# mbed92/soft-grip

Hardware: AMD Instinct MI355X
Metric: env steps/sec (whole node) at batch=4096 (higher is better)
Workload: dtype f64; 1 GPU; configs[2]: 4096 envs/GPU, softbox scene (nv=118), stiffness ~ U(300,1400), reference 200-step squeeze schedule from reset, 7 substeps per env step; 327 equality rows (composite neighbour equalities on: DESIGN.md 2, U2); volume tendon damper integrated explicitly; envs_per_gpu=4096, envs_flagged_bad=0

## Files before the change

soft-grip_amd/csrc/sg_phase.hip:

```cpp
#include "sg_work.h"

struct GenLds {
  StageRec2* stage;
  double* gas;
  double* gg;
  double* tmp;
  const double (*boxp)[3];
  const double (*boxm)[9];
  const ChainKin* K;
  const ChainLds2* cs;
  const double *qe, *ve, *asme, *we;
};

__device__ __forceinline__ void sg_gen_capsule(const SgPhaseArgs& a, const GenLds& L, int e, double* cp, double* cax) {
  const int N = a.nelem;
  auto EL = [&](int f, int k) { return a.elem[(size_t)f * N + k]; };
  const double dq = L.qe[e] - EL(SGE_QPOS0, e);
  cp[0] = EL(SGE_GX, e) + EL(SGE_AX, e) * dq; cp[1] = EL(SGE_GY, e) + EL(SGE_AY, e) * dq; cp[2] = EL(SGE_GZ, e) + EL(SGE_AZ, e) * dq;
  cax[0] = EL(SGE_CX, e); cax[1] = EL(SGE_CY, e); cax[2] = EL(SGE_CZ, e);
}

__device__ __noinline__ int sg_gen_phase(const SgPhaseArgs& a, const SgPlanHeader& H, const int env, const GenLds L, int* flags, int* touch) {
  const int lane = threadIdx.x, N = a.nelem;
  auto EL = [&](int f, int k) { return a.elem[(size_t)f * N + k]; };
// ... 621 lines not shown
              double fld[SG_RK];
#pragma unroll
              for (int q = 0; q < SG_RK; q++) fld[q] = 0.0;
              if (r < 3) {
#pragma unroll
                for (int d = 0; d < SG_CD; d++) fld[d] = c.Jf[r][d];
                fld[4] = c.Js[r]; fld[5] = c.b[r]; fld[6] = c.f[r];
                fld[7] = Afull[r][0] * c.f[0] + Afull[r][1] * c.f[1] + Afull[r][2] * c.f[2];
                fld[8] = Afull[r][0]; fld[9] = Afull[r][1]; fld[10] = Afull[r][2];
                fld[11] = c.invm * c.Js[r];
                fld[15] = c.R;
              } else {
                fld[0] = P11; fld[1] = P12; fld[2] = P22; fld[4] = __hiloint2double(0, sl);
                fld[8] = ee1; fld[9] = ee2; fld[10] = ecs; fld[11] = esn;
              }
              fld[12] = Wm[0][r]; fld[13] = Wm[1][r]; fld[14] = Wm[2][r];
#pragma unroll
              for (int pr = 0; pr < SG_RK / 2; pr++) fp[r][pr] = make_double2(fld[2 * pr], fld[2 * pr + 1]);
            }
          }
          if (!a.rowlayout) {
          double* ro = W.crec + SG_REC_INDEX(i, env / SG_EPW, 0, 2 * (env % SG_EPW) + half, nwb);
#pragma unroll
          for (int r = 0; r < 3; r++)
#pragma unroll
            for (int d = 0; d < SG_CD; d++) ro[(4 * r + d) * SG_SPW] = c.Jf[r][d];
#pragma unroll
          for (int r = 0; r < 3; r++) ro[(12 + r) * SG_SPW] = c.Js[r];
#pragma unroll
          for (int q = 0; q < 6; q++) ro[(15 + q) * SG_SPW] = c.A[q];
#pragma unroll
          for (int r = 0; r < 3; r++) ro[(21 + r) * SG_SPW] = c.b[r];
          ro[24 * SG_SPW] = c.R;
          ro[25 * SG_SPW] = c.invm;
#pragma unroll
          for (int r = 0; r < 3; r++) ro[(26 + r) * SG_SPW] = c.f[r];
          ((int*)(ro + 29 * SG_SPW))[0] = sl;
          }
        }
        const int nk = (ns0 > ns1 ? ns0 : ns1) - 32 * k;
        if (a.rowlayout && nk > 0) {
          const int nwb8 = (a.nenv + 7) / 8;
          const int li = lane & 31;
          auto X = [&](int sl_, int L) -> double2* {
            return (double2*)&Sm.stage[sl_ >> 4][32 * k] + ((sl_ & 15) * 8 + L);
          };
          __syncthreads();
          double2* const e0 = (double2*)&Sm.stage[li >> 4][32 * k] + ((li & 15) * 8 + 4 * half);
#pragma unroll
          for (int pr = 0; pr < SG_RK / 2; pr++) {
            e0[0] = fp[0][pr]; e0[1] = fp[1][pr]; e0[2] = fp[2][pr]; e0[3] = fp[3][pr];
            __syncthreads();
#pragma unroll
            for (int j = 0; j < 4; j++) {
              if (8 * j >= nk) break;
              const int e = j * 64 + lane, s_ = e >> 3, L = e & 7;
              if (s_ < nk) *(double2*)(W.crow + SG_ROW_INDEX(32 * k + s_, env >> 3, 2 * pr, 8 * (env & 7) + L, nwb8)) = *X(s_, L);
            }
            __syncthreads();
          }
        }
      }
      SG_T(5);
      double eqR[R], eqb[R], eqf[R];
      double tbp = 0, tjp = 0, tAp = 0;
#pragma unroll
      for (int r = 0; r < R; r++) {
        int e = r * 64 + lane;
        eqR[r] = 1; eqb[r] = 0; eqf[r] = 0;
        if (e < N) {
          double pos = qe[r] - EL(SGE_QPOS0, e), imp = impedance(H.eqj_solimp, pos, 0);
          eqR[r] = fmax(SG_MINVAL, (1 - imp) / imp * EL(SGE_INVW, e));
          double aref = -H.eqj_B * ve[r] - H.eqj_K * imp * pos;
          eqb[r] = asme[r] - aref;
          eqf[r] = -(we[r] - aref) / eqR[r];
          tbp += coef[r] * asme[r]; tjp += coef[r] * we[r]; tAp += coef[r] * coef[r] * invm[r];
        }
      }
      const int nnb = NB ? H.nnb : 0;
      constexpr int ND = NB ? 3 : 0;
      int nbe2[R][3], nbid[R][3];
      double nbc0[R][3];
      [[maybe_unused]] double nbff[R][3];
      [[maybe_unused]] double* const gnbf = W.nbf + (size_t)env * 3 * N;
#pragma unroll
      for (int r = 0; r < R; r++)
#pragma unroll
        for (int d = 0; d < 3; d++) { nbe2[r][d] = -1; nbid[r][d] = -1; nbc0[r][d] = 0; nbff[r][d] = 0; }
      if constexpr (NB) {
        const double im0 = 1.0 / (EL(SGE_MASS, 0) + EL(SGE_ARMATURE, 0));
        const SG_CONSTAS int* const cposc = (const SG_CONSTAS int*)a.cpos;
        const bool wantc = a.rowlayout && a.cst_rounds;
#pragma unroll
        for (int r = 0; r < R; r++) {
          const int e = r * 64 + lane;
          if (e < N) {
            double c4[4] = {0.0, 0.0, 0.0, 0.0};
            if (wantc) c4[0] = sg_div(im0, im0 + eqR[r]);
#pragma unroll
            for (int d = 0; d < 3; d++) {
              const int e2 = nbtabc[d * N + e];
              if (e2 >= 0) {
                const int id = nbtabc[(3 + d) * N + e];
                const double pos = (qe[r] - EL(SGE_QPOS0, e)) - (Sm.as[e2] - EL(SGE_QPOS0, e2)), imp = impedance(H.eqj_solimp, pos, 0);
                const double Rr = fmax(SG_MINVAL, (1 - imp) / imp * (EL(SGE_INVW, e) + EL(SGE_INVW, e2)));
                const double aref = -H.eqj_B * (ve[r] - Sm.ve[e2]) - H.eqj_K * imp * pos;
                const double bb = (asme[r] - Sm.asme[e2]) - aref, ff = -((we[r] - Sm.we[e2]) - aref) / Rr;
                nbe2[r][d] = e2; nbid[r][d] = id; nbc0[r][d] = ff * (0.5 * Rr * ff + bb);
                nbff[r][d] = ff; gnbf[id] = ff;
                W.nbb[(size_t)env * 3 * N + id] = bb; W.nbR[(size_t)env * 3 * N + id] = Rr;
                if (wantc) c4[1 + d] = sg_div(im0, 2.0 * im0 + Rr);
              }
            }
            if (wantc) {
              double* const dst = W.cst + SG_CST_INDEX(env >> 2, 0, 16 * (env & 3), a.cst_rounds) + cposc[e];
              *(double2*)dst = make_double2(c4[0], c4[1]);
              *(double2*)(dst + 2) = make_double2(c4[2], c4[3]);
            }
          }
        }
      }
      const double tpos = L0 - H.t0_L0, timp = impedance(H.eqt_solimp, tpos, 0), tR = fmax(SG_MINVAL, (1 - timp) / timp * H.eqt_invw);
      const double taref = -H.eqt_B * Ld - H.eqt_K * timp * tpos;
      const double tb = wave_sum2(tbp) - taref, tjar = wave_sum2(tjp) - taref, tA = wave_sum2(tAp) + tR;
      double tf = -tjar / tR;
      const int nmaxs = ns0 > ns1 ? ns0 : ns1;

      double aF[SG_CD];
      auto recompute_a = [&]() {
        __syncthreads();
#pragma unroll
        for (int r = 0; r < R; r++) {
          int e = r * 64 + lane;
          if (e < N) {
            double fe = eqf[r] + coef[r] * tf;
            if constexpr (NB) {
#pragma unroll
              for (int d = 0; d < 3; d++) if (nbid[r][d] >= 0) fe += nbff[r][d];
              double fin[3];
#pragma unroll
              for (int d = 0; d < 3; d++) { const int ii = nbtabc[(6 + d) * N + e]; fin[d] = ii >= 0 ? gnbf[ii] : 0.0; }
#pragma unroll
              for (int d = 0; d < 3; d++) fe -= fin[d];
            }
            double as_ = invm[r] * fe;
#pragma unroll
            for (int cb = 0; cb < SG_MAXCH * SG_CG; cb++) {
              const int u = Sm.eslot[e][cb], i0 = u & 0x3F, nst = u >> 6;
              if (nst >= 1) as_ += cval_at(cb / SG_CG, i0);
              if (nst >= 2) as_ += cval_at(cb / SG_CG, i0 + 1);
            }
            if constexpr (GEN)
              if (ngen) as_ += GL.gas[e];
            Sm.as[e] = as_;
          }
        }
        __syncthreads();
        double g[SG_CD] = {0, 0, 0, 0};
#pragma unroll
        for (int k = 0; k < CPL; k++)
#pragma unroll
          for (int d = 0; d < SG_CD; d++) g[d] += cg[k][d];
        if (is_chain_lane) {
          const int la = CS.lim_active;
#pragma unroll
          for (int k = 0; k < SG_MAXLIM; k++)
            if (la >> k & 1) g[k / 2] += CS.lim_sign[k] * CS.lim_f[k];
          if constexpr (GEN)
            if (ngen) {
#pragma unroll
              for (int d = 0; d < SG_CD; d++) g[d] += GL.gg[half * SG_CD + d];
            }
        }
#pragma unroll
        for (int d = 0; d < SG_CD; d++) {
          double x = g[d];
#pragma unroll
          for (int o = 16; o > 0; o >>= 1) x += __shfl_xor(x, o);
          g[d] = x;
        }
#pragma unroll
        for (int a2 = 0; a2 < SG_CD; a2++) {
          double s2 = 0;
#pragma unroll
          for (int b2 = 0; b2 < SG_CD; b2++) s2 += CS.Minv[4 * a2 + b2] * g[b2];
          aF[a2] = s2;
        }
        __syncthreads();
      };
      recompute_a();
      SG_T(6);
      {
        double cp = 0, tJap = 0;
#pragma unroll
        for (int r = 0; r < R; r++) {
          int e = r * 64 + lane;
          if (e < N) {
            double ae = Sm.as[e]; cp += eqf[r] * (0.5 * (ae + eqR[r] * eqf[r]) + eqb[r]); tJap += coef[r] * ae;
#pragma unroll
            for (int d = 0; d < ND; d++)
              if (nbid[r][d] >= 0) cp += 0.5 * nbff[r][d] * (ae - Sm.as[nbe2[r][d]]) + nbc0[r][d];
          }
        }
        double tJa = wave_sum2(tJap);
        if (lane == 0) cp += tf * (0.5 * (tJa + tR * tf) + tb);
        if (is_chain_lane) {
          const int la = CS.lim_active;
#pragma unroll
          for (int k = 0; k < SG_MAXLIM; k++)
            if (la >> k & 1) cp += CS.lim_f[k] * (0.5 * (CS.lim_sign[k] * aF[k / 2] + CS.lim_R[k] * CS.lim_f[k]) + CS.lim_b[k]);
        }
#pragma unroll
        for (int k = 0; k < CPL; k++)
          if ((lane & 31) + 32 * k < myn) {
            double as_ = csl_[k] >= 0 ? Sm.as[csl_[k]] : 0.0, ga = 0;
#pragma unroll
            for (int d = 0; d < SG_CD; d++) ga += cg[k][d] * aF[d];
            cp += 0.5 * (ga + cjsf[k] * as_) + ccost0[k];
          }
        [[maybe_unused]] double aF2[SG_MAXCH][SG_CD];
        if constexpr (GEN)
          if (ngen) {
#pragma unroll
            for (int d = 0; d < SG_CD; d++) {
              const double other = __shfl_xor(aF[d], 32);
              aF2[0][d] = high ? other : aF[d]; aF2[1][d] = high ? aF[d] : other;
            }
            cp += sg_gen_cost(a, env, ngen, aF2, Sm.as, 0);
          }
        double cost = wave_sum2(cp);
        if (cost > 0) {
          if constexpr (GEN)
            if (ngen) {
              sg_gen_cost(a, env, ngen, aF2, Sm.as, 1);
              for (int e = lane; e < N; e += 64) GL.gas[e] = 0.0;
              if (lane < SG_MAXCH * SG_CD) GL.gg[lane] = 0.0;
            }
#pragma unroll
          for (int r = 0; r < R; r++) {
            eqf[r] = 0;
#pragma unroll
            for (int d = 0; d < ND; d++) if (nbid[r][d] >= 0) { nbff[r][d] = 0.0; gnbf[nbid[r][d]] = 0.0; }
          }
          tf = 0;
          if (is_chain_lane) {
#pragma unroll
            for (int k = 0; k < SG_MAXLIM; k++) CS.lim_f[k] = 0;
          }
#pragma unroll
          for (int k = 0; k < CPL; k++) {
            int i = (lane & 31) + 32 * k;
            cjsf[k] = 0;
#pragma unroll
            for (int d = 0; d < SG_CD; d++) cg[k][d] = 0;
            if (i < myn) {
              cval_at(half, i) = 0.0;
              if (!a.rowlayout) {
              double* ro = W.crec + SG_REC_INDEX(i, env / SG_EPW, 0, 2 * (env % SG_EPW) + half, nwb);
#pragma unroll
              for (int r = 0; r < 3; r++) ro[(26 + r) * SG_SPW] = 0.0;
              }
              if (a.rowlayout) {
#pragma unroll
                for (int r = 0; r < 3; r++)
                  *(double2*)(W.crow + SG_ROW_INDEX(i, env >> 3, 6, 8 * (env & 7) + 4 * half + r, (a.nenv + 7) / 8)) = make_double2(0.0, 0.0);
              }
            }
          }
          __syncthreads();
          recompute_a();
        }
      }
      SG_T(7);
#pragma unroll
      for (int r = 0; r < R; r++) {
        int e = r * 64 + lane;
        if (e < N) {
          size_t o = (size_t)env * N + e;
          W.as[o] = Sm.as[e]; W.eqf[o] = eqf[r]; W.eqb[o] = eqb[r]; W.eqR[o] = eqR[r];
        }
      }
      if (is_chain_lane) {
        W.ns[st] = myn < SG_CAP ? myn : SG_CAP;
        W.lim_active[st] = CS.lim_active;
      }
      if (half < nchain) {
        static_assert(4 * SG_MAXLIM == 32, "one limit value per lane of a half");
        const int i = lane & 31;
        W.lim[(size_t)i * S + st] = (&CS.lim_sign[0])[i];
        if (i < SG_CD) W.saF[(size_t)i * S + st] = i == 0 ? aF[0] : (i == 1 ? aF[1] : (i == 2 ? aF[2] : aF[3]));
      }
      if (lane == 0) {
        W.envh[(size_t)0 * a.nenv + env] = tb; W.envh[(size_t)1 * a.nenv + env] = tR;
        W.envh[(size_t)2 * a.nenv + env] = tA; W.envh[(size_t)3 * a.nenv + env] = tf;
        W.shared[env] = shared_slider;
        W.pending[env] = 1;
        W.ncon[env] = ns0 + ns1 + ngen;
        W.gen[env] = ngen;
        W.nefc[env] = N + nnb + 1 + 3 * (ns0 + ns1 + ngen) + __popc(Sm.cs[0].lim_active) + (nchain > 1 ? __popc(Sm.cs[1].lim_active) : 0);
        W.touch[env] = touch;
      }
    }
  }

  SG_T(8);
  __syncthreads();
#pragma unroll
  for (int r = 0; r < R; r++) {
    int e = r * 64 + lane;
    if (e < N) { gq[e0 + e] = qe[r]; gv[e0 + e] = ve[r]; gw[e0 + e] = we[r]; }
  }
  if (lane == 0) {
    if (status | flags) atomicOr(&W.status[env], status | flags);
  }
  SG_T(9);
  SG_TEND();
}

#ifndef SG_X_PHASE_OCC
#define SG_X_PHASE_OCC 2
#endif
#ifndef SG_X_CPL
#define SG_X_CPL 2
#endif
template <int R, int CPL, bool NB, bool GEN = false>
__global__ __launch_bounds__(64, SG_X_PHASE_OCC) void sg_phase_kernel(SgPhaseArgs a) {
  if constexpr (GEN) {
    const int cnt = a.w.gen_count[0];
    a.do_finish = 0; a.do_reset = 0; a.sens = nullptr;
    for (int i = blockIdx.x; i < cnt && i < a.nenv; i += gridDim.x) {
      sg_phase_env<R, CPL, NB, true>(a, a.w.gen_list[i]);
      __syncthreads();
    }
  } else {
    sg_phase_env<R, CPL, NB, false>(a, blockIdx.x);
  }
}

__global__ __launch_bounds__(64) void sg_chain_kernel(SgPhaseArgs a) {
  const int lane = threadIdx.x, c = blockIdx.x & 1, env = (int)(blockIdx.x >> 1) * 64 + lane;
  if (blockIdx.x == 0 && lane == 0) a.w.gen_count[0] = 0;
  SG_T0();
  const SG_CONSTAS SgPlanHeader& H = *(const SG_CONSTAS SgPlanHeader*)a.H;
  const int nv = a.nv, nu = a.nu;
  const size_t S = 2 * (size_t)a.nenv;
  if (env >= a.nenv) return;
  const size_t st = 2 * (size_t)env + c;
  if (a.mask && !a.mask[env]) return;
  SgWork& W = a.w;
  if (a.first && c == 0) { W.status[env] = 0; if (!a.do_finish) W.pending[env] = 0; }
  if (c >= a.nchain) return;
  const int status = a.first ? 0 : W.status[env];
  const int pend = a.do_finish ? W.pending[env] : 0;
  const SgChain& C = H.chain[c];
  const double h = a.timestep;
  double* gq = a.qpos + (size_t)env * nv;
  double* gv = a.qvel + (size_t)env * nv;
  double* gw = a.warm + (size_t)env * nv;
  const double kenv = a.kenv[env];
  double q[SG_CD], v[SG_CD], w[SG_CD], kk[SG_CD], act = 0, ctrl = 0;
#pragma unroll
  for (int d = 0; d < SG_CD; d++) {
// ... 180 lines not shown
```

soft-grip_amd/csrc/sg_rows.hip:

```cpp
#include "sg_work.h"

template <int CTRL>
__device__ __forceinline__ double sg_dpp(double x) {
  int lo = __double2loint(x), hi = __double2hiint(x);
  lo = __builtin_amdgcn_update_dpp(0, lo, CTRL, 0xF, 0xF, true);
  hi = __builtin_amdgcn_update_dpp(0, hi, CTRL, 0xF, 0xF, true);
  return __hiloint2double(hi, lo);
}
template <int R_>
__device__ __forceinline__ double sg_qb(double x) { return sg_dpp<R_ * 0x55>(x); }
__device__ __forceinline__ double sg_qsum(double x) {
  x += sg_dpp<0xB1>(x);
  x += sg_dpp<0x4E>(x);
  return x;
}

__device__ __forceinline__ double sg_gsum8(double x) {
  x = sg_qsum(x);
  x += sg_dpp<0x141>(x);
  return x;
}

__device__ __forceinline__ double sg_gsum16(double x) {
  x = sg_gsum8(x);
  x += sg_dpp<0x140>(x);
  return x;
}

template <int NSL, int NB, int EPW>
__global__ __launch_bounds__(64) void sg_pgs_rows_kernel(SgPgsArgs a) {
  extern __shared__ double lds[];
  static_assert(!NB || EPW == 4, "neighbour-row models: four envs of 16 lanes per wavefront");
  constexpr bool CST = NB == 2;
  constexpr int LSH = NB ? 4 : 3, LPE = 1 << LSH;
  const int lane = threadIdx.x, le = lane >> LSH, g = lane & (LPE - 1), c = g >> 2, r = g & 3;
  const bool in_wave = le < EPW;
  const int lec = in_wave ? le : 0;
  const int env = blockIdx.x * EPW + le;
  const SG_CONSTAS SgPlanHeader& H = *(const SG_CONSTAS SgPlanHeader*)a.H;
  const int N = H.nelem;
  const size_t S = 2 * (size_t)a.nenv;
  const int nwb = (a.nenv + 7) / 8;
  const SgWork& W = a.w;
  const double mu0 = H.con_mu[0], mu1 = H.con_mu[1], pgs_scale = H.pgs_scale, tolerance = H.tolerance;
  const double mur = r == 1 ? mu0 : mu1;
  const double rsel0 = r == 0 ? 1.0 : 0.0, rsel1 = r == 1 ? 1.0 : 0.0, rsel2 = r == 2 ? 1.0 : 0.0;
  const int max_iter = H.iterations;
  unsigned pendmask = 0;
#pragma unroll
  for (int e2 = 0; e2 < EPW; e2++) {
    const int env2 = blockIdx.x * EPW + e2;
    pendmask |= (env2 < a.nenv && W.pending[env2 < a.nenv ? env2 : 0] != 0) ? 1u << e2 : 0u;
  }
  const bool valid = in_wave && ((pendmask >> lec) & 1u) != 0;
  if (pendmask == 0) return;
  constexpr int NR = 8 * NSL;
  constexpr int NA = NR + 8;
  const int NAr = SG_ROWS_NA_NB(N);
  const int GW = (CST ? 4 : 8) * (N + 1);
  double2* const AF = (double2*)lds + (size_t)lec * NR;
  double2* const BR = (double2*)lds + (size_t)EPW * NR + (size_t)lec * NR;
  double* const RI = lds + (size_t)4 * EPW * NR + (size_t)lec * NR;
  double2* const IC = (double2*)(lds + (size_t)5 * EPW * NR);
  double* const Ae = lds + (size_t)lec * NAr;
  double* const GS = lds + (size_t)EPW * NAr + (size_t)lec * GW;
  unsigned* const TAB = (unsigned*)(lds + (size_t)EPW * NAr + (size_t)EPW * GW);
  constexpr int TABW = CST ? 1 : 2;
  double* const Lnb = lds + (size_t)EPW * NAr + (size_t)EPW * GW + (size_t)8 * TABW * (H.eq_rounds + 8);
  double* Lzero = NB ? Lnb : lds + (size_t)(5 * EPW + 2) * NR;
  double* const Lenv = Lnb + 72;
  double* const ASb = NB ? Ae : (double*)AF;
  constexpr int ASS = NB ? 1 : 2;
  if (lane == 0) Lzero[0] = 0.0;
  if constexpr (!NB)
  for (int j = lane; j < NR; j += 64)
    IC[j] = j < N ? make_double2(1.0 / (a.elem[(size_t)SGE_MASS * N + j] + a.elem[(size_t)SGE_ARMATURE * N + j]), a.elem[(size_t)SGE_COEF * N + j]) : make_double2(0.0, 0.0);
#pragma unroll
  for (int e2 = 0; e2 < EPW; e2++) {
    const int env2 = blockIdx.x * EPW + e2;
    const bool v2 = ((pendmask >> e2) & 1u) != 0;
    if constexpr (!NB) {
      double2* const AF2 = (double2*)lds + (size_t)e2 * NR;
      double2* const BR2 = (double2*)lds + (size_t)EPW * NR + (size_t)e2 * NR;
      double* const RI2 = lds + (size_t)4 * EPW * NR + (size_t)e2 * NR;
#pragma unroll
      for (int j0 = 0; j0 < NR; j0 += 64) {
        const int j = j0 + lane;
        double2 af = make_double2(0.0, 0.0), br = make_double2(0.0, 1.0);
        double ri = 0.0;
        if (v2 && j < N) {
          const size_t o = (size_t)env2 * N + j;
          const double Rr = W.eqR[o], im = 1.0 / (a.elem[(size_t)SGE_MASS * N + j] + a.elem[(size_t)SGE_ARMATURE * N + j]);
          af = make_double2(W.as[o], W.eqf[o]); br = make_double2(W.eqb[o], Rr);
          ri = sg_div(1.0, im + Rr);
        }
        if (j < NR) { AF2[j] = af; BR2[j] = br; RI2[j] = ri; }
      }
    } else {
      double* const A2 = lds + (size_t)e2 * NAr;
      double ssum = 0.0;
#pragma unroll
      for (int j0 = 0; j0 < NA; j0 += 64) {
        const int j = j0 + lane;
        const double av = (v2 && j < N) ? W.as[(size_t)env2 * N + j] : 0.0;
        if (j < NAr) A2[j] = av;
        ssum += av;
      }
      ssum = wave_sum2(ssum);
      if (lane == 0) { Lenv[e2] = ssum; Lenv[EPW + e2] = 0.0; }
    }
  }
  if constexpr (NB) {
    [[maybe_unused]] const double im0s = 1.0 / (a.elem[(size_t)SGE_MASS * N] + a.elem[(size_t)SGE_ARMATURE * N]);
    constexpr int REC_TRIPS = (4 * (NR + 1) + 63) / 64;
#pragma unroll 4
    for (int t = 0; t < REC_TRIPS; t++) {
      const int u = lane + 64 * t;
      if (u >= 4 * (N + 1)) continue;
      const int e = u >> 2, d = u & 3, ec = e < N ? e : 0;
      const bool fix = d == 0;
      const int tabw = a.nbtab[(fix ? 0 : d - 1) * N + ec];
      const bool have = e < N && (fix || tabw >= 0);
      double bb[EPW], Rr[EPW], ff[EPW];
#pragma unroll
      for (int e2 = 0; e2 < EPW; e2++) {
        const int env2 = blockIdx.x * EPW + e2, envc = env2 < a.nenv ? env2 : 0;
        const size_t o = fix ? (size_t)envc * N + ec : (size_t)envc * 3 * N + (size_t)(d - 1) * N + ec;
        bb[e2] = (fix ? W.eqb : W.nbb)[o]; Rr[e2] = (fix ? W.eqR : W.nbR)[o]; ff[e2] = (fix ? W.eqf : W.nbf)[o];
      }
#pragma unroll
      for (int e2 = 0; e2 < EPW; e2++) {
        const int env2 = blockIdx.x * EPW + e2;
        const bool v2 = ((pendmask >> e2) & 1u) != 0;
        double* const GS2 = lds + (size_t)EPW * NAr + (size_t)e2 * GW;
        const double gg = (v2 && have) ? bb[e2] + Rr[e2] * ff[e2] : 0.0;
        if constexpr (CST) GS2[u] = gg;
        else ((double2*)GS2)[u] = make_double2(gg, (v2 && have) ? sg_div(im0s, (fix ? im0s : 2.0 * im0s) + Rr[e2]) : 0.0);
      }
    }
  }
  if constexpr (NB) {
    const int ntab = 16 * TABW * (H.eq_rounds + 8);
#pragma unroll 4
    for (int i = lane; i < ntab; i += 64) TAB[i] = a.tab[i];
  }
  const bool sv = valid && g < 8;
  const size_t st = 2 * (size_t)(sv ? env : 0) + (sv ? c : 0);
  int ns = 0, lim_active = 0, shared = 0;
  double Mrow[SG_CD] = {0, 0, 0, 0}, Mdiag[SG_CD] = {0, 0, 0, 0}, aFo = 0;
  double tb = 0, tR = 1, tA = 1, tf = 0;
  double lsign[SG_MAXLIM], lR[SG_MAXLIM], lb[SG_MAXLIM], lf[SG_MAXLIM];
#pragma unroll
  for (int k = 0; k < SG_MAXLIM; k++) { lsign[k] = 0; lR[k] = 1; lb[k] = 0; lf[k] = 0; }
  if (valid) {
    tb = W.envh[(size_t)0 * a.nenv + env]; tR = W.envh[(size_t)1 * a.nenv + env];
    tA = W.envh[(size_t)2 * a.nenv + env]; tf = W.envh[(size_t)3 * a.nenv + env];
    shared = W.shared[env];
  }
  const int ngen = valid ? W.gen[env] : 0;
  const bool wave_gen = __ballot(ngen > 0) != 0;
  if (sv) {
    ns = W.ns[st];
    lim_active = W.lim_active[st];
#pragma unroll
    for (int d = 0; d < SG_CD; d++) { Mrow[d] = W.sMinv[(size_t)(4 * r + d) * S + st]; Mdiag[d] = W.sMinv[(size_t)(5 * d) * S + st]; }
    aFo = W.saF[(size_t)r * S + st];
#pragma unroll
    for (int k = 0; k < SG_MAXLIM; k++) {
      lsign[k] = W.lim[((size_t)0 * SG_MAXLIM + k) * S + st]; lR[k] = W.lim[((size_t)1 * SG_MAXLIM + k) * S + st];
      lb[k] = W.lim[((size_t)2 * SG_MAXLIM + k) * S + st]; lf[k] = W.lim[((size_t)3 * SG_MAXLIM + k) * S + st];
    }
  }
  __syncthreads();
  int nsmax_v = ns;
#pragma unroll
  for (int o = 32; o > 0; o >>= 1) { int t = __shfl_xor(nsmax_v, o); nsmax_v = t > nsmax_v ? t : nsmax_v; }
  const int nsmax = __builtin_amdgcn_readfirstlane(nsmax_v);
  const unsigned long long any_lim = __ballot(lim_active != 0);

  bool running = valid;
  int iters = 0;
  double aoff = 0.0, Ssum = NB ? Lenv[lec] : 0.0, dS = 0.0;
  const double im0 = NB ? 1.0 / (a.elem[(size_t)SGE_MASS * N] + a.elem[(size_t)SGE_ARMATURE * N]) : 0.0;
  const bool has_row = sv;
  const double2* const row0 = has_row ? (const double2*)(W.crow + SG_ROW_INDEX(0, env >> 3, 8, 8 * (env & 7) + g, nwb))
                                      : (const double2*)(W.cdummy + ((size_t)blockIdx.x * (SG_RK / 2) + 4) * 128 + 2 * lane);
  const size_t slot_stride = has_row ? (size_t)(nwb + 2) * (SG_RK / 2) * 64 : 0;
  constexpr ptrdiff_t sink_off = 0;

  [[maybe_unused]] const double2* const cp0 = (const double2*)(W.cst + SG_CST_INDEX(blockIdx.x, 0, lane, H.eq_rounds + 8));
  [[maybe_unused]] double2 c0, c1, c2, c3;
  if constexpr (CST) { c0 = cp0[0]; c1 = cp0[64]; c2 = cp0[128]; c3 = cp0[192]; }
  SG_T0();
  for (int it = 0; it < max_iter; it++) {
    if (!__ballot(running)) break;
    SG_T(10);
    double imp_acc = 0;
    [[maybe_unused]] double tJap = 0;
    if constexpr (NB) {
      if (running) {
        char* const Ab = (char*)Ae;
        char* const Gb = (char*)GS;
        using TabW = std::conditional_t<CST, unsigned, uint2>;
        const TabW* tp = (const TabW*)TAB + g;
        const double2* cp = cp0;
        const int hh = g & 1;
        const double hm = hh ? 1.0 : 0.0, h0 = 1.0 - hm;
        const double Pfix = h0 * -aoff;
        double qc = 0.0, sc = 0.0;
        const int nrounds = H.eq_rounds;
        struct Adr { double *px, *py; double2* rec; };
        struct Off { double sA, wA, sB, wB, ga, gb; };
        auto adr_of = [&](const TabW tt) {
          Adr q;
          if constexpr (CST) { q.px = (double*)(Ab + (tt & 0x7ffu)); q.py = (double*)(Ab + ((tt >> 11) & 0x7ffu)); q.rec = (double2*)(Gb + ((tt >> 22) << 4)); }
          else { q.px = (double*)(Ab + (tt.x & 0xffffu)); q.py = (double*)(Ab + (tt.x >> 16)); q.rec = (double2*)(Gb + tt.y); }
          return q;
        };
        auto chain = [&](const Adr q, const double2 gg, const double2 cc, const double X, const double Y, Off& o) {
          const double cA = cc.x, cB = cc.y;
          const double PA = fma(X, hm, Pfix), dA = gg.x - PA, dB = gg.y - Y;
          const double sA0 = dA + X, O10 = X - cA * sA0, O20 = O10 - cB * (dB + O10);
          const double T = sg_dpp<0xB1>(O20);
          const double I = hh ? T : X;
          const double sA = dA + I, wA = cA * sA, O1 = I - wA, sB = dB + O1, wB = cB * sB, O2 = O1 - wB;
          const double PAn = fma(wA, hm, PA), Yn = Y + wB;
          const double e4 = sg_dpp<0xB1>(O2);
          *q.px = hh ? PAn : e4;
          *q.py = Yn;
          o.sA = sA; o.wA = wA; o.sB = sB; o.wB = wB; o.ga = PAn - O1; o.gb = Yn - O2;
        };
        auto offchain = [&](const Adr q, const Off& o) {
          qc += o.sA * o.wA + o.sB * o.wB;
          sc += o.wA * h0;
          if constexpr (CST) *q.rec = make_double2(o.ga, o.gb);
          else { q.rec[0].x = o.ga; q.rec[1].x = o.gb; }
        };
        auto ld_rec = [&](const Adr q, double2& gg, double2& cc) {
          if constexpr (CST) gg = *q.rec;
          else { const double2 ra = q.rec[0], rb = q.rec[1]; gg = make_double2(ra.x, rb.x); cc = make_double2(ra.y, rb.y); }
        };
        TabW tC = tp[0], tD = tp[16];
        Adr qA = adr_of(tC), qB = adr_of(tD);
        double2 gA, gB;
        ld_rec(qA, gA, c0); ld_rec(qB, gB, c1);
        double XA = *qA.px, YA = *qA.py, XB, YB;
        Off oA, oB;
        constexpr int TRIP = CST ? 4 : 2;
        const int P = (nrounds + TRIP - 1) & ~(TRIP - 1);
        for (int k = 0; k < P; k += TRIP) {
          [[maybe_unused]] const double2* const cpn = k + 4 < P ? cp + 256 : cp0;
#define SG_EQ_ROUND_PAIR(CA, CB, IA, IB, LA, LB)        \
          tp += 32;                                     \
          tC = tp[0]; tD = tp[16];                      \
          chain(qA, gA, CA, XA, YA, oA);                \
          if constexpr (CST) CA = cpn[IA];              \
          XB = *qB.px; YB = *qB.py;                     \
          __builtin_amdgcn_sched_barrier(0);            \
          offchain(qA, oA);                             \
          qA = adr_of(tC); ld_rec(qA, gA, LA);          \
          __builtin_amdgcn_sched_barrier(0);            \
          chain(qB, gB, CB, XB, YB, oB);                \
          if constexpr (CST) CB = cpn[IB];              \
          XA = *qA.px; YA = *qA.py;                     \
          __builtin_amdgcn_sched_barrier(0);            \
          offchain(qB, oB);                             \
          qB = adr_of(tD); ld_rec(qB, gB, LB);          \
          __builtin_amdgcn_sched_barrier(0);
          if constexpr (CST) {
            SG_EQ_ROUND_PAIR(c0, c1, 0, 64, c0, c1)
            SG_EQ_ROUND_PAIR(c2, c3, 128, 192, c2, c3)
          } else {
            SG_EQ_ROUND_PAIR(c0, c1, 0, 64, c0, c1)
          }
#undef SG_EQ_ROUND_PAIR
          cp = cpn;
// ... 398 lines not shown
```

soft-grip_amd/csrc/sg_work.h:

```cpp
#pragma once
#include <hip/hip_runtime.h>

#include "../../include/softgrip.h"
#include "sg_math.h"
#include "sg_general.h"

using namespace sgm;

#define SG_CAP 64
#define SG_NF 26
#define SG_RF 30
#define SG_REC_INDEX(slot, wave, field, pos, nwb) (((((size_t)(slot)) * ((nwb) + 1) + (wave)) * SG_RF + (field)) * SG_SPW + (pos))
#define SG_G 8
#define SG_EPW (64 / SG_G)
#define SG_SPW (2 * SG_EPW)
#define SG_GEN_GRID 256
#define SG_CHW 160

struct SgWork {
  double* crec;
  unsigned long long* secprof;
  double* crow;
  double* cdummy;
  int* ns;
  double* envh;
  int *shared, *pending, *status, *iters, *ncon, *nefc, *touch;
  double *sMinv, *saF;
  int* lim_active;
  double* lim;
  double *as, *eqf, *eqb, *eqR;
  double *asme, *fsm;
  double* chh;
  double *nbf, *nbb, *nbR;
  double* cst;
  double* gcon;
  int* gen;
  int* gen_count;
  int* gen_list;
  unsigned short* gpairs16;
  double* gcval;
};

struct SgPhaseArgs {
  const SgPlanHeader* H;
  const double* elem;
  double *qpos, *qvel, *warm, *act, *ctrl;
  const double* kenv;
  const int *kmask_jnt, *kmask_ten;
  const unsigned char* mask;
  double* sens;
  long long sens_stride;
  SgWork w;
  int nenv;
  int do_reset, do_finish, finish_integrate, do_begin, first;
  int rowlayout;
  const int* nbtab;
  const int* cpos;
  int cst_rounds;
  const SgGenPair* gpairs;
  int nelem, nv, nu, elem_dof0, nchain, t0_id;
  double timestep;
};

#define SG_RK 16
#define SG_CST_INDEX(w, k, l, rounds) ((((size_t)(w) * (rounds) + (k)) * 64 + (l)) * 2)
#define SG_ROW_INDEX(slot, wave, k, lane, nwb) \
  ((((((size_t)(slot)) * ((nwb) + 2) + (wave)) * (SG_RK / 2) + (k) / 2) * 64 + (lane)) * 2 + ((k) & 1))

__host__ __device__ constexpr int sg_rows_load_slot(int i, int ahead, int nsmax) { return i + ahead < nsmax ? i + ahead : -1; }

enum { SGH_QSM = 0, SGH_QFRC = 4, SGH_ACTDOT = 8, SGH_M = 9, SGH_K = 25, SGH_MINV = 73, SGH_V = 89, SGH_W = 93, SGH_BOX = 97,
       SGH_LIMACT = 121, SGH_LIMSIGN = 122, SGH_LIMR = 130, SGH_LIMB = 138, SGH_LIMF = 146 };

struct StageRec2 {
  double dist, pos[3], n[3];
  int sl, box;
};

struct ChainLds2 {
  double v[SG_CD], w[SG_CD], qacc_smooth[SG_CD], Minv[16];
  int lim_active, pad;
  double lim_sign[SG_MAXLIM], lim_R[SG_MAXLIM], lim_b[SG_MAXLIM], lim_f[SG_MAXLIM];
};

#define SG_PHASE_SLIM(R) ((R) >= 4)
#define SG_PAIRS_CAP(R) (SG_MAXCH * SG_CG * ((R) * 64 + 2))
template <int R, int CPL, bool NB>
struct Smem2 {
  ChainKin K[SG_MAXCH];
  ChainLds2 cs[SG_MAXCH];
  double boxp[SG_MAXCH * SG_CG][3], boxm[SG_MAXCH * SG_CG][9];
  double ve[R * 64], asme[R * 64], we[R * 64], as[R * 64];
  StageRec2 stage[SG_MAXCH][32 * CPL];
  unsigned short pairs[SG_PHASE_SLIM(R) ? 4 : SG_PAIRS_CAP(R)];
  unsigned char eslot[R * 64][SG_MAXCH * SG_CG];
  double cval[SG_PHASE_SLIM(R) ? 1 : SG_MAXCH * 32 * CPL];
};
#define SG_PAIR_CENTER 0xFFF

__device__ __forceinline__ double wave_sum2(double x) {
#pragma unroll
  for (int o = 32; o > 0; o >>= 1) x += __shfl_xor(x, o);
  return x;
}
__device__ __forceinline__ int lanes_below2(unsigned long long m) {
  return __builtin_amdgcn_mbcnt_hi((unsigned)(m >> 32), __builtin_amdgcn_mbcnt_lo((unsigned)m, 0));
}

#if defined(__HIP_DEVICE_COMPILE__)
#define SG_CONSTAS __attribute__((address_space(4)))
#else
#define SG_CONSTAS
#endif

#ifdef SG_SECTION_PROF
#define SG_T0() unsigned long long t_prev_ = __builtin_readcyclecounter(), t_acc_[26] = {0, 0, 0, 0, 0, 0, 0, 0, 0, 0, 0, 0, 0, 0, 0, 0, 0, 0, 0, 0, 0, 0, 0, 0, 0, 0}
#define SG_T(k)                                                   \
  do {                                                            \
    unsigned long long t_now_ = __builtin_readcyclecounter();     \
    t_acc_[k] += t_now_ - t_prev_;                                \
    t_prev_ = __builtin_readcyclecounter();                       \
  } while (0)
#define SG_TEND()                                                 \
  do {                                                            \
    if (threadIdx.x == 0)                                         \
      for (int k_ = 0; k_ < 26; k_++)                             \
        if (t_acc_[k_]) atomicAdd(&a.w.secprof[k_], t_acc_[k_]);  \
  } while (0)
#else
#define SG_T0()
#define SG_T(k)
#define SG_TEND()
#endif


struct SgPgsArgs {
  const unsigned* tab;
  const SgEqSlot* sched;
  const int* nbtab;
  const SgPlanHeader* H;
  const double* elem;
  SgWork w;
  int nenv;
};

#define SG_ROWS_LDS_FIX(EPW, NR) ((size_t)(5 * (EPW) + 2) * (NR) + 72)
#define SG_ROWS_NA_NB(N) (((N) + 2) & ~1)
#define SG_ROWS_LDS_NB(EPW, N, ROUNDS, CST) ((size_t)(EPW) * SG_ROWS_NA_NB(N) + (size_t)((CST) ? 4 : 8) * (EPW) * ((N) + 1) + (size_t)((CST) ? 8 : 16) * ((ROUNDS) + 8) + 72 + 2 * (EPW))
// ... 13 lines not shown
```

Baseline: 1.126 million env-steps/s.

## Precompute neighbour-row g and c terms in phase kernel and batch rows-kernel prologue loads

The phase kernel now writes the combined b+R*f value and the im0/(im0+R) coefficient directly in a per-element interleaved layout (nb index = (env*N+e)*3+d), instead of storing b, R and f separately for the rows kernel to recombine. The rows kernel prologue for neighbour models issues all global loads up front (as values, g/c records, env and quad scalars, first table batch) behind a sched_barrier, then writes them to LDS, and applies neutral values afterwards via selects instead of branches. Early exit when no env is pending is dropped for NB models. This is meant to cut global traffic and load latency in the prologue, at the cost of more registers, loads for invalid envs, and an extra nbb rewrite when cost>0 zeroes forces.

```diff
diff --git a/soft-grip_amd/csrc/sg_phase.hip b/soft-grip_amd/csrc/sg_phase.hip
--- a/soft-grip_amd/csrc/sg_phase.hip
+++ b/soft-grip_amd/csrc/sg_phase.hip
@@ -727,21 +727,22 @@
       int nbe2[R][3], nbid[R][3];
       double nbc0[R][3];
       [[maybe_unused]] double nbff[R][3];
+      [[maybe_unused]] double nbbb[R][3];
       [[maybe_unused]] double* const gnbf = W.nbf + (size_t)env * 3 * N;
 #pragma unroll
       for (int r = 0; r < R; r++)
 #pragma unroll
-        for (int d = 0; d < 3; d++) { nbe2[r][d] = -1; nbid[r][d] = -1; nbc0[r][d] = 0; nbff[r][d] = 0; }
+        for (int d = 0; d < 3; d++) { nbe2[r][d] = -1; nbid[r][d] = -1; nbc0[r][d] = 0; nbff[r][d] = 0; nbbb[r][d] = 0; }
       if constexpr (NB) {
         const double im0 = 1.0 / (EL(SGE_MASS, 0) + EL(SGE_ARMATURE, 0));
         const SG_CONSTAS int* const cposc = (const SG_CONSTAS int*)a.cpos;
-        const bool wantc = a.rowlayout && a.cst_rounds;
+        const bool ready = a.rowlayout != 0, wantc = ready && a.cst_rounds;
 #pragma unroll
         for (int r = 0; r < R; r++) {
           const int e = r * 64 + lane;
           if (e < N) {
-            double c4[4] = {0.0, 0.0, 0.0, 0.0};
-            if (wantc) c4[0] = sg_div(im0, im0 + eqR[r]);
+            double c4[4] = {0.0, 0.0, 0.0, 0.0}, g3[3] = {0.0, 0.0, 0.0};
+            if (ready) c4[0] = sg_div(im0, im0 + eqR[r]);
 #pragma unroll
             for (int d = 0; d < 3; d++) {
               const int e2 = nbtabc[d * N + e];
@@ -753,8 +754,19 @@
                 const double bb = (asme[r] - Sm.asme[e2]) - aref, ff = -((we[r] - Sm.we[e2]) - aref) / Rr;
                 nbe2[r][d] = e2; nbid[r][d] = id; nbc0[r][d] = ff * (0.5 * Rr * ff + bb);
                 nbff[r][d] = ff; gnbf[id] = ff;
-                W.nbb[(size_t)env * 3 * N + id] = bb; W.nbR[(size_t)env * 3 * N + id] = Rr;
-                if (wantc) c4[1 + d] = sg_div(im0, 2.0 * im0 + Rr);
+                nbbb[r][d] = bb;
+                if (ready) { g3[d] = fma(Rr, ff, bb); c4[1 + d] = sg_div(im0, 2.0 * im0 + Rr); }
+                else { W.nbb[(size_t)env * 3 * N + id] = bb; W.nbR[(size_t)env * 3 * N + id] = Rr; }
+              }
+            }
+            if (ready) {
+              const size_t o3 = sg_eq_nb_index((size_t)env, e, 0, N);
+#pragma unroll
+              for (int d = 0; d < 3; d++) W.nbb[o3 + d] = g3[d];
+              if (!wantc) {
+                W.eqR[sg_eq_fix_index((size_t)env, e, N)] = c4[0];
+#pragma unroll
+                for (int d = 0; d < 3; d++) W.nbR[o3 + d] = c4[1 + d];
               }
             }
             if (wantc) {
@@ -885,7 +897,11 @@
           for (int r = 0; r < R; r++) {
             eqf[r] = 0;
 #pragma unroll
-            for (int d = 0; d < ND; d++) if (nbid[r][d] >= 0) { nbff[r][d] = 0.0; gnbf[nbid[r][d]] = 0.0; }
+            for (int d = 0; d < ND; d++)
+              if (nbid[r][d] >= 0) {
+                nbff[r][d] = 0.0; gnbf[nbid[r][d]] = 0.0;
+                if (a.rowlayout) W.nbb[sg_eq_nb_index((size_t)env, r * 64 + lane, d, N)] = nbbb[r][d];
+              }
           }
           tf = 0;
           if (is_chain_lane) {
@@ -922,7 +938,9 @@
         int e = r * 64 + lane;
         if (e < N) {
           size_t o = (size_t)env * N + e;
-          W.as[o] = Sm.as[e]; W.eqf[o] = eqf[r]; W.eqb[o] = eqb[r]; W.eqR[o] = eqR[r];
+          W.as[o] = Sm.as[e];
+          if (NB && a.rowlayout) W.eqb[o] = fma(eqR[r], eqf[r], eqb[r]);
+          else { W.eqf[o] = eqf[r]; W.eqb[o] = eqb[r]; W.eqR[o] = eqR[r]; }
         }
       }
       if (is_chain_lane) {
diff --git a/soft-grip_amd/csrc/sg_rows.hip b/soft-grip_amd/csrc/sg_rows.hip
--- a/soft-grip_amd/csrc/sg_rows.hip
+++ b/soft-grip_amd/csrc/sg_rows.hip
@@ -30,6 +30,7 @@
 template <int NSL, int NB, int EPW>
 __global__ __launch_bounds__(64) void sg_pgs_rows_kernel(SgPgsArgs a) {
   extern __shared__ double lds[];
+  SG_T0();
   static_assert(!NB || EPW == 4, "neighbour-row models: four envs of 16 lanes per wavefront");
   constexpr bool CST = NB == 2;
   constexpr int LSH = NB ? 4 : 3, LPE = 1 << LSH;
@@ -47,13 +48,19 @@
   const double rsel0 = r == 0 ? 1.0 : 0.0, rsel1 = r == 1 ? 1.0 : 0.0, rsel2 = r == 2 ? 1.0 : 0.0;
   const int max_iter = H.iterations;
   unsigned pendmask = 0;
-#pragma unroll
-  for (int e2 = 0; e2 < EPW; e2++) {
-    const int env2 = blockIdx.x * EPW + e2;
-    pendmask |= (env2 < a.nenv && W.pending[env2 < a.nenv ? env2 : 0] != 0) ? 1u << e2 : 0u;
+  {
+    int pw[EPW];
+#pragma unroll
+    for (int e2 = 0; e2 < EPW; e2++) {
+      const int env2 = blockIdx.x * EPW + e2;
+      pw[e2] = W.pending[env2 < a.nenv ? env2 : a.nenv - 1];
+    }
+#pragma unroll
+    for (int e2 = 0; e2 < EPW; e2++) pendmask |= ((int)(blockIdx.x * EPW + e2 < a.nenv) & (int)(pw[e2] != 0)) ? 1u << e2 : 0u;
   }
   const bool valid = in_wave && ((pendmask >> lec) & 1u) != 0;
-  if (pendmask == 0) return;
+  if constexpr (!NB)
+    if (pendmask == 0) return;
   constexpr int NR = 8 * NSL;
   constexpr int NA = NR + 8;
   const int NAr = SG_ROWS_NA_NB(N);
@@ -75,11 +82,11 @@
   if constexpr (!NB)
   for (int j = lane; j < NR; j += 64)
     IC[j] = j < N ? make_double2(1.0 / (a.elem[(size_t)SGE_MASS * N + j] + a.elem[(size_t)SGE_ARMATURE * N + j]), a.elem[(size_t)SGE_COEF * N + j]) : make_double2(0.0, 0.0);
-#pragma unroll
-  for (int e2 = 0; e2 < EPW; e2++) {
-    const int env2 = blockIdx.x * EPW + e2;
-    const bool v2 = ((pendmask >> e2) & 1u) != 0;
-    if constexpr (!NB) {
+  if constexpr (!NB) {
+#pragma unroll
+    for (int e2 = 0; e2 < EPW; e2++) {
+      const int env2 = blockIdx.x * EPW + e2;
+      const bool v2 = ((pendmask >> e2) & 1u) != 0;
       double2* const AF2 = (double2*)lds + (size_t)e2 * NR;
       double2* const BR2 = (double2*)lds + (size_t)EPW * NR + (size_t)e2 * NR;
       double* const RI2 = lds + (size_t)4 * EPW * NR + (size_t)e2 * NR;
@@ -96,70 +103,22 @@
         }
         if (j < NR) { AF2[j] = af; BR2[j] = br; RI2[j] = ri; }
       }
-    } else {
-      double* const A2 = lds + (size_t)e2 * NAr;
-      double ssum = 0.0;
-#pragma unroll
-      for (int j0 = 0; j0 < NA; j0 += 64) {
-        const int j = j0 + lane;
-        const double av = (v2 && j < N) ? W.as[(size_t)env2 * N + j] : 0.0;
-        if (j < NAr) A2[j] = av;
-        ssum += av;
-      }
-      ssum = wave_sum2(ssum);
-      if (lane == 0) { Lenv[e2] = ssum; Lenv[EPW + e2] = 0.0; }
-    }
-  }
-  if constexpr (NB) {
-    [[maybe_unused]] const double im0s = 1.0 / (a.elem[(size_t)SGE_MASS * N] + a.elem[(size_t)SGE_ARMATURE * N]);
-    constexpr int REC_TRIPS = (4 * (NR + 1) + 63) / 64;
-#pragma unroll 4
-    for (int t = 0; t < REC_TRIPS; t++) {
-      const int u = lane + 64 * t;
-      if (u >= 4 * (N + 1)) continue;
-      const int e = u >> 2, d = u & 3, ec = e < N ? e : 0;
-      const bool fix = d == 0;
-      const int tabw = a.nbtab[(fix ? 0 : d - 1) * N + ec];
-      const bool have = e < N && (fix || tabw >= 0);
-      double bb[EPW], Rr[EPW], ff[EPW];
-#pragma unroll
-      for (int e2 = 0; e2 < EPW; e2++) {
-        const int env2 = blockIdx.x * EPW + e2, envc = env2 < a.nenv ? env2 : 0;
-        const size_t o = fix ? (size_t)envc * N + ec : (size_t)envc * 3 * N + (size_t)(d - 1) * N + ec;
-        bb[e2] = (fix ? W.eqb : W.nbb)[o]; Rr[e2] = (fix ? W.eqR : W.nbR)[o]; ff[e2] = (fix ? W.eqf : W.nbf)[o];
-      }
-#pragma unroll
-      for (int e2 = 0; e2 < EPW; e2++) {
-        const int env2 = blockIdx.x * EPW + e2;
-        const bool v2 = ((pendmask >> e2) & 1u) != 0;
-        double* const GS2 = lds + (size_t)EPW * NAr + (size_t)e2 * GW;
-        const double gg = (v2 && have) ? bb[e2] + Rr[e2] * ff[e2] : 0.0;
-        if constexpr (CST) GS2[u] = gg;
-        else ((double2*)GS2)[u] = make_double2(gg, (v2 && have) ? sg_div(im0s, (fix ? im0s : 2.0 * im0s) + Rr[e2]) : 0.0);
-      }
-    }
-  }
-  if constexpr (NB) {
-    const int ntab = 16 * TABW * (H.eq_rounds + 8);
-#pragma unroll 4
-    for (int i = lane; i < ntab; i += 64) TAB[i] = a.tab[i];
+    }
   }
   const bool sv = valid && g < 8;
-  const size_t st = 2 * (size_t)(sv ? env : 0) + (sv ? c : 0);
-  int ns = 0, lim_active = 0, shared = 0;
-  double Mrow[SG_CD] = {0, 0, 0, 0}, Mdiag[SG_CD] = {0, 0, 0, 0}, aFo = 0;
-  double tb = 0, tR = 1, tA = 1, tf = 0;
+  const int envl = env < a.nenv ? env : a.nenv - 1;
+  const size_t st = 2 * (size_t)envl + (c & 1);
+  int ns, lim_active, shared, ngen;
+  double Mrow[SG_CD], Mdiag[SG_CD], aFo;
+  double tb, tR, tA, tf;
   double lsign[SG_MAXLIM], lR[SG_MAXLIM], lb[SG_MAXLIM], lf[SG_MAXLIM];
-#pragma unroll
-  for (int k = 0; k < SG_MAXLIM; k++) { lsign[k] = 0; lR[k] = 1; lb[k] = 0; lf[k] = 0; }
-  if (valid) {
-    tb = W.envh[(size_t)0 * a.nenv + env]; tR = W.envh[(size_t)1 * a.nenv + env];
-    tA = W.envh[(size_t)2 * a.nenv + env]; tf = W.envh[(size_t)3 * a.nenv + env];
-    shared = W.shared[env];
-  }
-  const int ngen = valid ? W.gen[env] : 0;
-  const bool wave_gen = __ballot(ngen > 0) != 0;
-  if (sv) {
+  auto env_loads = [&]() {
+    tb = W.envh[(size_t)0 * a.nenv + envl]; tR = W.envh[(size_t)1 * a.nenv + envl];
+    tA = W.envh[(size_t)2 * a.nenv + envl]; tf = W.envh[(size_t)3 * a.nenv + envl];
+    shared = W.shared[envl];
+    ngen = W.gen[envl];
+  };
+  auto quad_loads = [&]() {
     ns = W.ns[st];
     lim_active = W.lim_active[st];
 #pragma unroll
@@ -170,7 +129,103 @@
       lsign[k] = W.lim[((size_t)0 * SG_MAXLIM + k) * S + st]; lR[k] = W.lim[((size_t)1 * SG_MAXLIM + k) * S + st];
       lb[k] = W.lim[((size_t)2 * SG_MAXLIM + k) * S + st]; lf[k] = W.lim[((size_t)3 * SG_MAXLIM + k) * S + st];
     }
+  };
+  auto neutral_unless = [&](const bool ve, const bool vq) {
+    tb = ve ? tb : 0.0; tR = ve ? tR : 1.0; tA = ve ? tA : 1.0; tf = ve ? tf : 0.0;
+    shared = ve ? shared : 0; ngen = ve ? ngen : 0;
+    ns = vq ? ns : 0; lim_active = vq ? lim_active : 0;
+#pragma unroll
+    for (int d = 0; d < SG_CD; d++) { Mrow[d] = vq ? Mrow[d] : 0.0; Mdiag[d] = vq ? Mdiag[d] : 0.0; }
+    aFo = vq ? aFo : 0.0;
+#pragma unroll
+    for (int k = 0; k < SG_MAXLIM; k++) { lsign[k] = vq ? lsign[k] : 0.0; lR[k] = vq ? lR[k] : 1.0; lb[k] = vq ? lb[k] : 0.0; lf[k] = vq ? lf[k] : 0.0; }
+  };
+  auto env_neutral = [&]() { tb = 0; tR = 1; tA = 1; tf = 0; shared = 0; ngen = 0; };
+  auto quad_neutral = [&]() {
+    ns = 0; lim_active = 0; aFo = 0;
+#pragma unroll
+    for (int d = 0; d < SG_CD; d++) { Mrow[d] = 0; Mdiag[d] = 0; }
+#pragma unroll
+    for (int k = 0; k < SG_MAXLIM; k++) { lsign[k] = 0; lR[k] = 1; lb[k] = 0; lf[k] = 0; }
+  };
+  if constexpr (NB) {
+    constexpr int ATRIPS = (NA + 63) / 64, REC_TRIPS = sg_eq_rec_trips(NR);
+    constexpr int TAB_BATCH = 4;
+    const int ntab4 = 4 * TABW * (H.eq_rounds + 8);
+    double av[EPW][ATRIPS], gv[EPW][REC_TRIPS];
+    [[maybe_unused]] double cv[EPW][REC_TRIPS];
+    uint4 tw[TAB_BATCH];
+#pragma unroll
+    for (int e2 = 0; e2 < EPW; e2++) {
+      const int env2 = blockIdx.x * EPW + e2;
+      const double* const as2 = W.as + (size_t)(env2 < a.nenv ? env2 : a.nenv - 1) * N;
+#pragma unroll
+      for (int k = 0; k < ATRIPS; k++) { const int j = 64 * k + lane; av[e2][k] = as2[j < N ? j : N - 1]; }
+    }
+#pragma unroll
+    for (int t = 0; t < REC_TRIPS; t++) {
+      const int u = sg_eq_rec_row(lane, t);
+      const bool fix = ((u < 4 * N ? u : 4 * N - 1) & 3) == 0;
+#pragma unroll
+      for (int e2 = 0; e2 < EPW; e2++) {
+        const size_t o = sg_eq_rec_index((size_t)(blockIdx.x * EPW + e2), u, N, (size_t)a.nenv);
+        gv[e2][t] = (fix ? W.eqb : W.nbb)[o];
+        if constexpr (!CST) cv[e2][t] = (fix ? W.eqR : W.nbR)[o];
+      }
+    }
+    env_loads();
+    quad_loads();
+#pragma unroll
+    for (int q = 0; q < TAB_BATCH; q++) { const int i = lane + 64 * q; tw[q] = ((const uint4*)a.tab)[i < ntab4 ? i : ntab4 - 1]; }
+    __builtin_amdgcn_sched_barrier(0);
+    double ssum[EPW];
+#pragma unroll
+    for (int e2 = 0; e2 < EPW; e2++) {
+      double* const A2 = lds + (size_t)e2 * NAr;
+      ssum[e2] = 0.0;
+#pragma unroll
+      for (int k = 0; k < ATRIPS; k++) {
+        const int j = 64 * k + lane;
+        const double v = j < N ? av[e2][k] : 0.0;
+        A2[j < NAr ? j : NAr - 1] = v;
+        ssum[e2] += v;
+      }
+    }
+#pragma unroll
+    for (int o = 32; o > 0; o >>= 1) {
+      double t_[EPW];
+#pragma unroll
+      for (int e2 = 0; e2 < EPW; e2++) t_[e2] = __shfl_xor(ssum[e2], o);
+#pragma unroll
+      for (int e2 = 0; e2 < EPW; e2++) ssum[e2] += t_[e2];
+    }
+#pragma unroll
+    for (int e2 = 0; e2 < EPW; e2++) {
+      *(lane == 0 ? &Lenv[e2] : &Lzero[1 + lane]) = ssum[e2];
+      *(lane == 0 ? &Lenv[EPW + e2] : &Lzero[1 + lane]) = 0.0;
+    }
+#pragma unroll
+    for (int t = 0; t < REC_TRIPS; t++) {
+      const int u = sg_eq_rec_row(lane, t);
+      const bool live = sg_eq_rec_live(u, N);
+      const int us = sg_eq_rec_stored(u, N) ? u : 4 * (N + 1) - 1;
+#pragma unroll
+      for (int e2 = 0; e2 < EPW; e2++) {
+        double* const GS2 = lds + (size_t)EPW * NAr + (size_t)e2 * GW;
+        if constexpr (CST) GS2[us] = live ? gv[e2][t] : 0.0;
+        else ((double2*)GS2)[us] = make_double2(live ? gv[e2][t] : 0.0, live ? cv[e2][t] : 0.0);
+      }
+    }
+#pragma unroll
+    for (int q = 0; q < TAB_BATCH; q++) { const int i = lane + 64 * q; ((uint4*)TAB)[i < ntab4 ? i : ntab4 - 1] = tw[q]; }
+    for (int i = lane + 64 * TAB_BATCH; i < ntab4; i += 64) ((uint4*)TAB)[i] = ((const uint4*)a.tab)[i];
+    neutral_unless(valid, sv);
+  } else {
+    env_neutral(); quad_neutral();
+    if (valid) env_loads();
+    if (sv) quad_loads();
   }
+  const bool wave_gen = __ballot(ngen > 0) != 0;
   __syncthreads();
   int nsmax_v = ns;
 #pragma unroll
@@ -191,7 +246,7 @@
   [[maybe_unused]] const double2* const cp0 = (const double2*)(W.cst + SG_CST_INDEX(blockIdx.x, 0, lane, H.eq_rounds + 8));
   [[maybe_unused]] double2 c0, c1, c2, c3;
   if constexpr (CST) { c0 = cp0[0]; c1 = cp0[64]; c2 = cp0[128]; c3 = cp0[192]; }
-  SG_T0();
+  SG_T(25);
   for (int it = 0; it < max_iter; it++) {
     if (!__ballot(running)) break;
     SG_T(10);
diff --git a/soft-grip_amd/csrc/sg_work.h b/soft-grip_amd/csrc/sg_work.h
--- a/soft-grip_amd/csrc/sg_work.h
+++ b/soft-grip_amd/csrc/sg_work.h
@@ -64,6 +64,17 @@
 
 #define SG_RK 16
 #define SG_CST_INDEX(w, k, l, rounds) ((((size_t)(w) * (rounds) + (k)) * 64 + (l)) * 2)
+__host__ __device__ constexpr size_t sg_eq_fix_index(size_t env, int e, int N) { return env * (size_t)N + (size_t)e; }
+__host__ __device__ constexpr size_t sg_eq_nb_index(size_t env, int e, int d, int N) { return (env * (size_t)N + (size_t)e) * 3 + (size_t)d; }
+__host__ __device__ constexpr int sg_eq_rec_trips(int nr) { return (4 * (nr + 1) + 63) / 64; }
+__host__ __device__ constexpr int sg_eq_rec_row(int lane, int trip) { return lane + 64 * trip; }
+__host__ __device__ constexpr bool sg_eq_rec_stored(int u, int N) { return u < 4 * (N + 1); }
+__host__ __device__ constexpr bool sg_eq_rec_live(int u, int N) { return u < 4 * N; }
+__host__ __device__ constexpr size_t sg_eq_rec_index(size_t env, int u, int N, size_t nenv) {
+  const size_t envc = env < nenv ? env : nenv - 1;
+  const int uc = u < 4 * N ? u : 4 * N - 1, e = uc >> 2, d = uc & 3;
+  return d == 0 ? sg_eq_fix_index(envc, e, N) : sg_eq_nb_index(envc, e, d - 1, N);
+}
 #define SG_ROW_INDEX(slot, wave, k, lane, nwb) \
   ((((((size_t)(slot)) * ((nwb) + 2) + (wave)) * (SG_RK / 2) + (k) / 2) * 64 + (lane)) * 2 + ((k) & 1))
 
```

After: 1.140 million env-steps/s (median of 6 runs). 1.01x the previous value.
